# antoyang/TubeDETR

Hardware: AMD Instinct MI355X
Metric: training clips/sec (fwd+bwd) at T=100 k=4 res=352, 1/2/4/8 MI355X (higher is better)
Workload: dtype bf16

## Files before the change

### tubedetr_amd/csrc/gemm_conv.hip

```cpp
#include <stdlib.h>

#include "gemm_dev.h"
#include "gemm_host.h"

#ifndef TD_BIG_XCD_CONTIG
#define TD_BIG_XCD_CONTIG 1
#endif
namespace td {

struct GemmParams {
  const char* src;
  const char* w;
  char* out;
  td_conv_desc d;
  int M, K;
  uint32_t src_bytes, w_bytes;
  unsigned long long* dbg;
  const float* bias;
  const char* residual;
  const char* mask_src;
  int relu, sigmoid;
  float alpha;
  uint32_t drop_thresh;
  float drop_scale;
// ... 933 lines not shown
      const int row = it * RPI + rsub;
      const int sw = row & (CPRW - 1);
      float v[EPL];
#pragma unroll
      for (int q = 0; q < EPL / 4; ++q) {
        const float4 f = *(const float4*)(stg + row * WN + (((cc * (EPL / 4) + q) ^ sw) * 4));
        v[4 * q + 0] = f.x + bias[4 * q + 0]; v[4 * q + 1] = f.y + bias[4 * q + 1];
        v[4 * q + 2] = f.z + bias[4 * q + 2]; v[4 * q + 3] = f.w + bias[4 * q + 3];
      }
      if (p.residual) {
        float r8[EPL];
        unpack16<T>(res[b][it], r8);
#pragma unroll
        for (int r = 0; r < EPL; ++r) v[r] += r8[r];
      }
      if (p.relu) {
#pragma unroll
        for (int r = 0; r < EPL; ++r) v[r] = fmaxf(v[r], 0.f);
      }
      if (p.mask_src) {
        float m8[EPL];
        unpack16<T>(msk[b][it], m8);
#pragma unroll
        for (int r = 0; r < EPL; ++r) v[r] = m8[r] > 0.f ? v[r] : 0.f;
      }
      if (live[b][it]) st16(p.out + offs[b][it] * ES, pack16<T>(v));
    }
    asm volatile("s_waitcnt lgkmcnt(0)" ::: "memory");
  }
  TD_STAMP(5);
#undef TD_STAMP
}

template <int NKT, bool RES, bool MSK>
__global__ __launch_bounds__(256, 2) void pw_resident2_kernel(GemmParams p, int MT, int P) {
  using T = u16;
  constexpr int ES = 2;
  constexpr uint32_t OOB = 0xFFFFFFF0u;
  constexpr int WM = 32, WN = 64, TM = 2, TN = 4;
  constexpr int CPRW = WN / 4, EPL = 8, LPR = WN / EPL, RPI = 64 / LPR, NIT = WM / RPI;
  constexpr int NOPS = NIT * ((RES ? 1 : 0) + (MSK ? 1 : 0));
  constexpr bool AHEAD = NOPS > 0 && !(RES && MSK && NKT == 4);
  constexpr int NA = 2 * NKT;
  constexpr int AUX_NT = (TD_NT & 2) ? 2 : 0;
  __shared__ __attribute__((aligned(16))) char sA0[32768];
  __shared__ __attribute__((aligned(16))) char sA1[32768];
  __shared__ __attribute__((aligned(16))) char sT[4 * 16 * WN * 4];
  const td_conv_desc& d = p.d;
  const int t = threadIdx.x;
  const int wave = __builtin_amdgcn_readfirstlane(t >> 6), lane = t & 63;
  const int NT = d.Nc >> 7;
  const int xcd = blockIdx.x & 7, local = blockIdx.x >> 3;
  const int GPX = P / NT;
  const int nt = local % NT, gl = local / NT;
  if (gl >= GPX) return;
  const int gid = xcd * GPX + gl, G = 8 * GPX;
  const int lrow = lane >> 3, chunk = (lane & 7) ^ lrow;
  const uint32_t out_bytes = (uint32_t)p.M * (uint32_t)d.ldc * ES;
  const __amdgpu_buffer_rsrc_t rs_src = __builtin_amdgcn_make_buffer_rsrc((void*)p.src, 0, p.src_bytes, 0x00020000);
  const __amdgpu_buffer_rsrc_t rs_out = __builtin_amdgcn_make_buffer_rsrc((void*)p.out, 0, out_bytes, 0x00020000);
  const __amdgpu_buffer_rsrc_t rs_res = __builtin_amdgcn_make_buffer_rsrc((void*)(RES ? p.residual : p.out), 0, out_bytes, 0x00020000);
  const __amdgpu_buffer_rsrc_t rs_msk = __builtin_amdgcn_make_buffer_rsrc((void*)(MSK ? p.mask_src : p.out), 0, out_bytes, 0x00020000);
  const int n0 = nt * 128;
  const int HoWo = d.Ho * d.Wo;
  const bool strided = d.stride != 1;
  auto issue_A = [&](char* buf, int mt) {
    const int m0 = mt * 64;
// ... 60 lines not shown
#pragma unroll
      for (int j = 0; j < TM; ++j) acc[i][j] = f32x4{0.f, 0.f, 0.f, 0.f};
#pragma unroll
    for (int kt = 0; kt < NKT; ++kt)
#pragma unroll
      for (int ks = 0; ks < 2; ++ks) {
        const int cidx = ks * 4 + lg;
        uint4 af[TM];
#pragma unroll
        for (int j = 0; j < TM; ++j) {
          const int row = wy * WM + j * 16 + lr;
          af[j] = *(const uint4*)(cur + kt * 8192 + row * 128 + ((cidx ^ (row & 7)) << 4));
        }
#pragma unroll
        for (int i = 0; i < TN; ++i)
#pragma unroll
          for (int j = 0; j < TM; ++j) Mfma<T>::run(wfr[kt][ks][i], af[j], acc[i][j]);
      }
    asm volatile("s_waitcnt lgkmcnt(0)" ::: "memory");
    __builtin_amdgcn_s_barrier();
    issue_A(cur, mt + 2 * G);
    if constexpr (AHEAD) fetch_ops(mt + G, B ^ 1);
    if constexpr (NOPS > 0) {
      wait_vmcnt<NA + (AHEAD ? NOPS : 0)>();
      __builtin_amdgcn_sched_barrier(0);
    }
    constexpr int RB = AHEAD ? B : 0;
#pragma unroll
    for (int j = 0; j < TM; ++j) {
#pragma unroll
      for (int i = 0; i < TN; ++i) {
        const int c = (i * 4 + lg) ^ (lr & (CPRW - 1));
        const f32x4 a = acc[i][j];
        *(float4*)(stg + lr * WN + c * 4) = make_float4(a[0], a[1], a[2], a[3]);
      }
      asm volatile("s_waitcnt lgkmcnt(0)" ::: "memory");
#pragma unroll
      for (int h = 0; h < 16 / RPI; ++h) {
        const int it = j * (16 / RPI) + h;
        const int row = h * RPI + rsub;
        const int sw = row & (CPRW - 1);
        float v[EPL];
#pragma unroll
        for (int q = 0; q < EPL / 4; ++q) {
          const float4 f = *(const float4*)(stg + row * WN + (((cc * (EPL / 4) + q) ^ sw) * 4));
          v[4 * q + 0] = f.x + bias[4 * q + 0]; v[4 * q + 1] = f.y + bias[4 * q + 1];
          v[4 * q + 2] = f.z + bias[4 * q + 2]; v[4 * q + 3] = f.w + bias[4 * q + 3];
        }
        const uint32_t off = seg_off(mt, it);
        if constexpr (RES) {
          float r8[EPL];
          unpack16<T>(make_uint4(res[RB][it].x, res[RB][it].y, res[RB][it].z, res[RB][it].w), r8);
#pragma unroll
          for (int r = 0; r < EPL; ++r) v[r] += r8[r];
        }
        if (p.relu) {
#pragma unroll
          for (int r = 0; r < EPL; ++r) v[r] = fmaxf(v[r], 0.f);
        }
        if constexpr (MSK) {
          float m8[EPL];
          unpack16<T>(make_uint4(msk[RB][it].x, msk[RB][it].y, msk[RB][it].z, msk[RB][it].w), m8);
#pragma unroll
          for (int r = 0; r < EPL; ++r) v[r] = m8[r] > 0.f ? v[r] : 0.f;
        }
        if (p.drop_thresh) {
#pragma unroll
// ... 4 lines not shown
      }
      asm volatile("s_waitcnt lgkmcnt(0)" ::: "memory");
    }
  };

  int mt = gid;
  issue_A(sA0, mt);
  issue_A(sA1, mt + G);
  if constexpr (AHEAD) fetch_ops(mt, 0);
  while (mt < MT) {
    step(sA0, sA1, mt, ic<0>{});
    mt += G;
    if (mt >= MT) break;
    step(sA1, sA0, mt, ic<1>{});
    mt += G;
  }
  asm volatile("s_waitcnt vmcnt(0)" ::: "memory");
}

}

using namespace td;


static thread_local unsigned long long* g_dbg = nullptr;
extern "C" int td_debug_set_stamp_buffer(unsigned long long* buf) { g_dbg = buf; return TD_OK; }
unsigned long long* td::stamp_buffer() { return g_dbg; }

const GemmKnobs& td::gemm_knobs() {
  static const GemmKnobs knobs = [] {
    GemmKnobs k;
    const struct { const char* name; int* value; } vars[] = {
        {"TD_PW_PERSIST", &k.pw_persist}, {"TD_PW_PERSIST_MIN", &k.pw_persist_min}, {"TD_PW_PERSIST_DROPOUT", &k.pw_persist_dropout},
        {"TD_CONV_TAP_UNIFORM", &k.conv_tap_uniform}, {"TD_CONV_BIG", &k.conv_big}, {"TD_CONV_BIG_MIN_WG", &k.conv_big_min_wg},
        {"TD_CONV_TAP_INNER", &k.conv_tap_inner}, {"TD_CONV_BIG_PERSIST", &k.conv_big_persist}, {"TD_CONV_DEEP", &k.conv_deep},
        {"TD_DGRAD_S2_PARITY", &k.dgrad_s2_parity}, {"TD_WGRAD_BLOCKS", &k.wgrad_blocks}, {"TD_WGRAD_WIDE", &k.wgrad_wide},
        {"TD_WGRAD_WIDE_MIN_M", &k.wgrad_wide_min_m}, {"TD_WGRAD_SPLIT_STAGES", &k.wgrad_split_stages}};
    for (const auto& v : vars)
      if (const char* e = getenv(v.name)) *v.value = atoi(e);
    return k;
  }();
  return knobs;
}

static int fill_epilogue(GemmParams& p, const td_epilogue* e, const char* who) {
  p.alpha = 1.f;
  if (!e) return TD_OK;
  p.bias = e->bias;
  p.residual = (const char*)e->residual;
  p.mask_src = (const char*)e->mask_src;
  p.relu = e->relu;
  p.sigmoid = e->sigmoid;
  if (e->alpha != 0.f) p.alpha = e->alpha;
  if (e->dropout_p > 0.f) {
    TD_REQUIRE(e->dropout_p < 1.f, "%s: dropout_p must be < 1", who);
    p.drop_thresh = dropout_threshold(e->dropout_p);
    p.drop_scale = 1.f / (1.f - e->dropout_p);
    p.seed = e->dropout_seed;
    p.seed_dev = e->dropout_counter;
  }
  return TD_OK;
}

typedef void (*GemmKernel)(GemmParams);
typedef void (*PersistentKernel)(GemmParams, int, int);
template <typename T, int BM, int BN, int NST>
static GemmKernel tiled_instance(int walk) {
  switch (walk) {
    case TD_GEMM_WALK_POINTWISE: return conv_gemm_kernel<T, BM, BN, NST, true>;
    case TD_GEMM_WALK_TAP_UNIFORM: return conv_gemm_kernel<T, BM, BN, NST, false, true>;
    case TD_GEMM_WALK_GATHER: return conv_gemm_kernel<T, BM, BN, NST, false>;
    default: return conv_gemm_kernel<T, BM, BN, 2, true, false, true>;
  }
}
template <int NKT>
static PersistentKernel persistent_instance(bool res, bool msk) {
  if (res) return msk ? pw_resident2_kernel<NKT, true, true> : pw_resident2_kernel<NKT, true, false>;
  return msk ? pw_resident2_kernel<NKT, false, true> : pw_resident2_kernel<NKT, false, false>;
}

static int launch_route(const GemmRoute& r, GemmParams& p, hipStream_t st) {
  const bool bf16 = r.dtype == TD_BF16, tu = r.walk == TD_GEMM_WALK_TAP_UNIFORM;
  GemmKernel k = nullptr;
  PersistentKernel kp = nullptr;
  switch (r.kernel) {
    case TD_GEMM_KERNEL_PERSISTENT:
      kp = r.nkt == 1 ? persistent_instance<1>(r.res, r.msk) : r.nkt == 2 ? persistent_instance<2>(r.res, r.msk) :
           r.nkt == 3 ? persistent_instance<3>(r.res, r.msk) : persistent_instance<4>(r.res, r.msk);
      break;
    case TD_GEMM_KERNEL_BIG8:
      if (tu) k = r.res ? conv_gemm_big8_kernel<true, true> : conv_gemm_big8_kernel<true, false>;
      else k = r.res ? conv_gemm_big8_kernel<false, true> : conv_gemm_big8_kernel<false, false>;
      break;
    case TD_GEMM_KERNEL_BIG8N: k = tu ? conv_gemm_big8n_kernel<true> : conv_gemm_big8n_kernel<false>; break;
    default:
      if (r.bn == 64) k = bf16 ? tiled_instance<u16, 128, 64, 2>(r.walk) : tiled_instance<float, 128, 64, 2>(r.walk);
      else if (r.stages == 3) k = tiled_instance<u16, 64, 128, 3>(r.walk);
      else if (r.bm == 64) k = bf16 ? tiled_instance<u16, 64, 128, 2>(r.walk) : tiled_instance<float, 64, 128, 2>(r.walk);
      else k = bf16 ? tiled_instance<u16, 128, 128, 2>(r.walk) : tiled_instance<float, 128, 128, 2>(r.walk);
  }
  const bool prof = prof_on();
  if (prof) {
    prof_begin(r.family, r.dtype, 2.0 * r.M * r.N * r.K, st, r.M, r.N, r.K, r.R, r.stride, r.mode);
    prof_set_bytes(r.bytes);
  }
  if (kp) kp<<<r.grid, r.block, 0, st>>>(p, r.MTp, r.Pp);
  else k<<<r.grid, r.block, 0, st>>>(p);
  if (prof) prof_end(st);
  return check_launch(r.label);
}

static int conv_gemm_launch(const void* src, const void* wmat, void* out, const td_conv_desc* d, const td_epilogue* e, int dtype, int n_cu,
                            const WeightSubset* sub, td_stream_t stream, td_gemm_route* report) {
  GemmRoute r;
  int rc = plan_conv_launch(d, epi_flags(e), dtype, n_cu, gemm_knobs(), sub, r);
  if (rc) return rc;
  GemmParams p;
  memset(&p, 0, sizeof(p));
  rc = fill_epilogue(p, e, "td_conv_gemm");
  if (rc) return rc;
  if (report) {
// ... 21 lines not shown

static int conv_gemm_call(const void* src, const void* wmat, void* out, const td_conv_desc* d, const td_epilogue* e, int dtype, int n_cu,
                          td_stream_t stream, td_gemm_route* report, int* n_report) {
  const bool split = conv_splits_by_parity(d, e, dtype, gemm_knobs());
  if (n_report) *n_report = split ? 4 : 1;
  if (!split) return conv_gemm_launch(src, wmat, out, d, e, dtype, n_cu, nullptr, stream, report);
  int rc = validate(d, dtype, "td_conv_gemm");
  for (int i = 0; i < 4 && !rc; ++i) {
    const ParityClass c = parity_class(d, i >> 1, i & 1);
    td_epilogue ec;
    memset(&ec, 0, sizeof(ec));
    if (e) ec = *e;
    if (ec.residual) ec.residual = (const char*)ec.residual + c.out_off;
    if (ec.mask_src) ec.mask_src = (const char*)ec.mask_src + c.out_off;
    if (report) rc = conv_gemm_launch(nullptr, nullptr, nullptr, &c.d, &ec, dtype, n_cu, &c.sub, stream, report + i);
    else rc = conv_gemm_launch(src, (const char*)wmat + c.w_off, (char*)out + c.out_off, &c.d, &ec, dtype, n_cu, &c.sub, stream, nullptr);
  }
  return rc;
}

extern "C" int td_conv_gemm(const void* src, const void* wmat, void* out, const td_conv_desc* d, const td_epilogue* e,
                            int dtype, td_stream_t stream) {
  TD_REQUIRE(src && wmat && out && d, "td_conv_gemm: null pointer");
  return conv_gemm_call(src, wmat, out, d, e, dtype, cu_count(), stream, nullptr, nullptr);
}

extern "C" int td_conv_gemm_route(const td_conv_desc* d, const td_epilogue* e, int dtype, int n_cu, td_gemm_route* routes, int* n_routes) {
  TD_REQUIRE(d && routes && n_routes, "td_conv_gemm: null pointer");
  TD_REQUIRE(n_cu >= 1, "td_conv_gemm_route: n_cu=%d", n_cu);
  return conv_gemm_call(nullptr, nullptr, nullptr, d, e, dtype, n_cu, nullptr, routes, n_routes);
}

static int linear_ex_call(const void* a1, const void* a2, const void* wmat, void* out, const td_linear_ex_desc* x, bool has_a2, const td_epilogue* e,
                          int dtype, td_stream_t stream, td_gemm_route* report) {
  GemmRoute r;
  int rc = plan_linear_ex(x, has_a2, epi_flags(e), dtype, r);
  if (rc) return rc;
  GemmParams p;
  memset(&p, 0, sizeof(p));
  rc = fill_epilogue(p, e, "td_linear_ex");
  if (rc) return rc;
  if (report) {
    *report = r;
    return TD_OK;
  }
  p.src = (const char*)a1;
  p.src2 = (const char*)a2;
  p.w = (const char*)wmat;
  p.out = (char*)out;
  p.M = r.M;
  p.K = r.K;
  p.K1 = x->K1;
  p.lda1 = x->lda1;
  p.lda2 = a2 ? x->lda2 : 0;
  p.ldr = x->ldr > 0 ? x->ldr : x->ldc;
  p.w_shared = (a2 && x->w_shared) ? 1 : 0;
  p.a1_map = x->a1_map;
  p.a2_map = a2 ? x->a2_map : nullptr;
  p.out_map = x->out_map;
  p.res_map = x->res_map;
  p.d.N = 1; p.d.Hs = x->M; p.d.Ws = 1; p.d.C = p.K; p.d.Ho = x->M; p.d.Wo = 1; p.d.R = p.d.S = 1; p.d.stride = 1; p.d.Nc = x->N; p.d.ldc = x->ldc; p.d.out_sp = 1;
  p.src_bytes = r.src_bytes;
  p.src2_bytes = r.src2_bytes;
  p.w_bytes = r.w_bytes;
  return launch_route(r, p, (hipStream_t)stream);
}

extern "C" int td_linear_ex(const void* a1, const void* a2, const void* wmat, void* out, const td_linear_ex_desc* x, const td_epilogue* e,
                            int dtype, td_stream_t stream) {
  TD_REQUIRE(a1 && wmat && out && x, "td_linear_ex: null pointer");
  return linear_ex_call(a1, a2, wmat, out, x, a2 != nullptr, e, dtype, stream, nullptr);
}

extern "C" int td_linear_ex_route(const td_linear_ex_desc* x, int has_a2, const td_epilogue* e, int dtype, int n_cu, td_gemm_route* routes, int* n_routes) {
  TD_REQUIRE(x && routes && n_routes, "td_linear_ex: null pointer");
  (void)n_cu;
  *n_routes = 1;
  return linear_ex_call(nullptr, nullptr, nullptr, nullptr, x, has_a2 != 0, e, dtype, nullptr, routes);
}
```

### tubedetr_amd/csrc/gemm_route.h

```cpp
#pragma once
#include <stdint.h>
#include <string.h>

#include "../../include/tubedetr_hip.h"

#ifndef TD_REQUIRE
namespace td {
void set_error(const char* fmt, ...);
inline int cdiv(int a, int b) { return (a + b - 1) / b; }
}
#define TD_REQUIRE(cond, ...)           \
  do {                                  \
    if (!(cond)) {                      \
      td::set_error(__VA_ARGS__);       \
      return TD_ERR_INVALID;            \
    }                                   \
  } while (0)
#endif

namespace td {

struct GemmKnobs {
  int pw_persist = 1;
  int pw_persist_min = 4;
  int pw_persist_dropout = 1;
  int conv_tap_uniform = 1;
  int conv_big = 1;
  int conv_big_min_wg = 160;
  int conv_tap_inner = 1;
  int conv_big_persist = 1;
  int conv_deep = 1;
  int dgrad_s2_parity = 1;
  int wgrad_blocks = 256, wgrad_wide = 1, wgrad_wide_min_m = 4096, wgrad_split_stages = 0;
};

struct WeightSubset {
  int w_ld;
  int ntap;
  int wtap[4];
  size_t w_bytes;
};

struct EpiFlags {
  bool res, msk, sigmoid, drop;
  float alpha;
};
inline EpiFlags epi_flags(const td_epilogue* e) {
  EpiFlags f = {false, false, false, false, 1.f};
  if (e) f = {e->residual != nullptr, e->mask_src != nullptr, e->sigmoid != 0, e->dropout_p > 0.f, e->alpha != 0.f ? e->alpha : 1.f};
  return f;
}

struct GemmRoute : td_gemm_route {
  bool res, msk;
  int nkt, MTp, Pp;
  int tap_inner;
  uint32_t src_bytes, src2_bytes, w_bytes;
  double bytes;
  const char* label;
};

inline int validate(const td_conv_desc* d, int dtype, const char* who) {
  const int vec = dtype == TD_BF16 ? 8 : 4;
  TD_REQUIRE(dtype == TD_F32 || dtype == TD_BF16, "%s: bad dtype %d", who, dtype);
  TD_REQUIRE(d->C % vec == 0, "%s: source channels C=%d must be a multiple of %d (pad them)", who, d->C, vec);
  TD_REQUIRE(d->N > 0 && d->Hs > 0 && d->Ws > 0 && d->Ho > 0 && d->Wo > 0 && d->R > 0 && d->S > 0 && d->stride > 0,
             "%s: bad geometry", who);
  TD_REQUIRE((double)d->N * d->Hs * d->Ws * d->C < 2147483647.0, "%s: source tensor exceeds 2^31 elements", who);
  TD_REQUIRE(!d->aniso || (d->mode == 0 && d->stride_w >= 1 && d->pad_w >= 0 && d->out_sp <= 1), "%s: anisotropic stride / padding is a forward-only geometry", who);
  return TD_OK;
}

inline void tiled_shape(GemmRoute& r) {
  const bool narrow = r.N <= 64;
  const int tiles128 = cdiv(r.M, 128) * cdiv(r.N, 128);
  const bool small_m = !narrow && (tiles128 < 512 || r.K <= 512);
  r.kernel = TD_GEMM_KERNEL_TILED;
  r.family = narrow ? TD_PROF_GEMM_128x64 : (small_m ? TD_PROF_GEMM_64x128 : TD_PROF_GEMM_128x128);
  r.bm = small_m ? 64 : 128;
  r.bn = narrow ? 64 : 128;
  r.stages = 2;
  r.grid = 8 * cdiv(cdiv(r.M, r.bm), 8) * cdiv(r.N, r.bn);
  r.block = 256;
}

inline int plan_conv_launch(const td_conv_desc* d, const EpiFlags& f, int dtype, int n_cu, const GemmKnobs& kn, const WeightSubset* sub, GemmRoute& r) {
  int rc = validate(d, dtype, "td_conv_gemm");
// ... 66 lines not shown
  return TD_OK;
}

inline bool conv_splits_by_parity(const td_conv_desc* d, const td_epilogue* e, int dtype, const GemmKnobs& kn) {
  return kn.dgrad_s2_parity && dtype == TD_BF16 && d->mode == 1 && d->stride == 2 && d->R == 3 && d->S == 3 && d->pad == 1 && !d->aniso && d->out_sp <= 1 &&
         d->Ho == 2 * d->Hs && d->Wo == 2 * d->Ws && d->C % 64 == 0 && d->ldc >= d->Nc && !(e && (e->dropout_p > 0.f || e->sigmoid));
}
struct ParityClass {
  td_conv_desc d;
  WeightSubset sub;
  size_t w_off, out_off;
};
inline ParityClass parity_class(const td_conv_desc* d, int ph, int pw) {
  const int Hg = d->Hs, Wg = d->Ws, Co = d->C, H = d->Ho, W = d->Wo;
  const size_t es = 2, wbytes = (size_t)d->Nc * 9 * Co * es;
  const int nr = ph ? 2 : 1, ns = pw ? 2 : 1;
  const int rmap[2] = {ph ? 2 : 1, 0}, smap[2] = {pw ? 2 : 1, 0};
  ParityClass c;
  memset(&c, 0, sizeof(c));
  c.d = {d->N, Hg, Wg, Co, Hg, Wg, nr, ns, 1, 0, 0, d->Nc, d->ldc, 2, H, W};
  c.sub.w_ld = 9 * Co;
  c.sub.ntap = nr * ns;
  for (int r = 0; r < nr; ++r)
    for (int s_ = 0; s_ < ns; ++s_) c.sub.wtap[r * ns + s_] = rmap[r] * 3 + smap[s_];
  c.out_off = ((size_t)ph * W + pw) * d->ldc * es;
  if (c.sub.ntap == 1) {
    c.w_off = (size_t)c.sub.wtap[0] * Co * es;
    c.sub.wtap[0] = 0;
  }
  c.sub.w_bytes = wbytes - c.w_off;
  return c;
}

inline int plan_linear_ex(const td_linear_ex_desc* x, bool has_a2, const EpiFlags& f, int dtype, GemmRoute& r) {
  TD_REQUIRE(dtype == TD_F32 || dtype == TD_BF16, "td_linear_ex: bad dtype %d", dtype);
  const int vec = dtype == TD_BF16 ? 8 : 4, bk = dtype == TD_BF16 ? 64 : 32;
  const int es = dtype == TD_BF16 ? 2 : 4;
  const int K2 = has_a2 ? x->K2 : 0;
  TD_REQUIRE(x->M >= 1 && x->N >= 1 && x->K1 >= vec && K2 >= 0, "td_linear_ex: bad sizes");
  TD_REQUIRE(x->K1 % vec == 0 && K2 % vec == 0 && x->lda1 % vec == 0 && (!has_a2 || x->lda2 % vec == 0), "td_linear_ex: K1 / K2 / lda must be multiples of %d", vec);
  TD_REQUIRE(!has_a2 || x->K1 % bk == 0, "td_linear_ex: with a second source K1=%d must be a multiple of the K tile (%d)", x->K1, bk);
  TD_REQUIRE(x->lda1 >= x->K1 && (!has_a2 || x->lda2 >= K2) && x->ldc >= x->N, "td_linear_ex: row stride smaller than the row");
  TD_REQUIRE(x->rows1 >= 1 && (!has_a2 || x->rows2 >= 1) && (x->a1_map || x->rows1 >= x->M) && (!has_a2 || x->a2_map || x->rows2 >= x->M),
             "td_linear_ex: source has fewer rows than M and no row map");
  const bool w_shared = has_a2 && x->w_shared;
  TD_REQUIRE(!w_shared || K2 == x->K1, "td_linear_ex: a shared weight needs K2 == K1");
  memset(&r, 0, sizeof(r));
  r.dtype = dtype; r.M = x->M; r.N = x->N; r.K = x->K1 + K2; r.R = 1; r.stride = 1; r.mode = 2;
  const double b1 = (double)x->rows1 * x->lda1 * es, b2 = has_a2 ? (double)x->rows2 * x->lda2 * es : 16.0, wb = (double)x->N * (w_shared ? x->K1 : r.K) * es;
  TD_REQUIRE(b1 < 4294967000.0 && b2 < 4294967000.0 && wb < 4294967000.0, "td_linear_ex: operand exceeds the 4 GiB buffer-descriptor range");
  r.src_bytes = (uint32_t)b1;
  r.src2_bytes = (uint32_t)b2;
  r.w_bytes = (uint32_t)wb;
  r.res = f.res;
  r.msk = f.msk;
  tiled_shape(r);
  r.walk = TD_GEMM_WALK_GX;
  r.bytes = ((double)r.M * r.K + (double)r.N * r.K + (double)r.M * r.N * (1 + f.res + f.msk)) * es;
  r.label = "td_linear_ex";
  return TD_OK;
}

}
```

### tubedetr_amd/csrc/resnet_exec.hip

```cpp
#include <stdlib.h>

#include <algorithm>
#include <vector>

#include "td_common.h"

namespace td {

struct ConvSpec {
  int cin, cout, k, stride, pad;
};
struct Tens {
  size_t off;
  int H, W, C;
};
struct BlockPlan {
  int conv[4];
  int stride, stage;
  Tens in, h1, h2, idt, out;
};
struct Plan {
  std::vector<ConvSpec> convs;
  std::vector<BlockPlan> blocks;
  Tens x, stem, pool;
// ... 64 lines not shown
      t->off = off;
      off += bytes(*t);
    } else {
      t->off = (size_t)(ring % 6) * maxb;
      ++ring;
    }
  }
  P.total = save ? off : 6 * maxb;
  Tens prev = P.pool;
  for (auto& b : P.blocks) {
    b.in = prev;
    prev = b.out;
  }
  return P;
}

struct FrameGroups {
  double lim_elems;
  int N;
  FrameGroups(int N_, int H, int W, int es) : N(N_) {
    lim_elems = std::min(2147483647.0, 4294963200.0 / es);
    if (const char* e = getenv("TD_TRUNK_MAX_FRAMES")) lim_elems = std::min(lim_elems, atof(e) * 16.0 * H * W);
  }
  int step(size_t per_frame) const {
    const long long nmax = std::max(1LL, (long long)(lim_elems / (double)per_frame));
    if (N <= nmax) return N;
    const long long groups = (N + nmax - 1) / nmax;
    return (int)((N + groups - 1) / groups);
  }
};
static inline size_t frame_elems(const Tens& t) { return (size_t)t.H * t.W * t.C; }

static int run_conv(const char* ws, const Tens& in, const Tens& out, int N, const ConvSpec& c, const void* w, const float* bias,
                    const char* residual, int relu, int dtype, td_stream_t st, const FrameGroups* fg = nullptr) {
  const int es = dtype == TD_BF16 ? 2 : 4;
  const int step = fg ? fg->step(std::max(frame_elems(in), frame_elems(out))) : N;
  for (int f0 = 0; f0 < N; f0 += step) {
    const int n = std::min(step, N - f0);
    td_conv_desc d = {n, in.H, in.W, in.C, out.H, out.W, c.k, c.k, c.stride, c.pad, 0, c.cout, c.cout, 1, 0, 0};
    td_epilogue e;
    memset(&e, 0, sizeof(e));
    e.bias = bias;
    e.residual = residual ? residual + (size_t)f0 * frame_elems(out) * es : nullptr;
    e.relu = relu;
    int rc = td_conv_gemm(ws + in.off + (size_t)f0 * frame_elems(in) * es, w, (void*)(ws + out.off + (size_t)f0 * frame_elems(out) * es), &d, &e, dtype, st);
    if (rc) return rc;
  }
  return TD_OK;
}

}
using namespace td;

extern "C" size_t td_resnet_fwd_ws_bytes(int N, int H, int W, const int* nblocks, int dtype, int save) {
  return make_plan(N, H, W, nblocks, dtype, save).total;
}

extern "C" int td_resnet_num_convs(const int* nblocks) {
  int n = 1;
  for (int s = 0; s < 4; ++s) n += 3 * nblocks[s] + (nblocks[s] > 0 ? 1 : 0);
  return n;
}

extern "C" int td_resnet_fwd(const td_frame_source* srcs, int n_srcs, const float* mean, const float* inv_std, int N, int H, int W,
                             const int* nblocks, const void* const* w_fwd, const float* const* bias, int save, void* ws,
                             size_t ws_bytes, void** feat, int* feat_hw, int stem_pairs, int first_train_stage, int dtype, td_stream_t stream) {
  TD_REQUIRE(srcs && n_srcs >= 1 && nblocks && w_fwd && bias && ws && feat, "td_resnet_fwd: null pointer");
  TD_REQUIRE(dtype == TD_F32 || dtype == TD_BF16, "td_resnet_fwd: bad dtype");
  {
    long long tot = 0;
    for (int i = 0; i < n_srcs; ++i) tot += srcs[i].n;
    TD_REQUIRE(tot == N, "td_resnet_fwd: the sources contribute %lld frames, N = %d", tot, N);
  }
  Plan P = make_plan(N, H, W, nblocks, dtype, save);
  TD_REQUIRE(ws_bytes >= P.total, "td_resnet_fwd: workspace too small (%zu < %zu)", ws_bytes, P.total);
  char* base = (char*)ws;
  int rc;
  const FrameGroups groups(N, H, W, P.es);
  const FrameGroups* fg = save ? nullptr : &groups;
  bool stem_done = false;
  if (stem_pairs) {
    TD_REQUIRE(dtype == TD_BF16 && (W & 1) == 0, "td_resnet_fwd: the pixel-pair stem needs bf16 and an even frame width");
    rc = td_frames_to_nhwc(srcs, n_srcs, 3, H, W, 4, mean, inv_std, base + P.x.off, dtype, stream);
    if (rc) return rc;
    static const int fused = [] { const char* e_ = getenv("TD_STEM_FUSED"); return e_ ? atoi(e_) : 1; }();
    if (fused) {
      rc = td_stem_pool(base + P.x.off, w_fwd[0], bias[0], base + P.pool.off, N, H, W, dtype, stream);
      stem_done = true;
    } else {
      const int step = fg ? fg->step(frame_elems(P.stem)) : N;
      for (int f0 = 0; f0 < N && !rc; f0 += step) {
        td_conv_desc d = {std::min(step, N - f0), H, W / 2, 8, P.stem.H, P.stem.W, 7, 4, 2, 3, 0, 64, 64, 1, 0, 0, 1, 1, 2};
        td_epilogue e;
        memset(&e, 0, sizeof(e));
        e.bias = bias[0];
        e.relu = 1;
        rc = td_conv_gemm(base + P.x.off + (size_t)f0 * H * W * 4 * P.es, w_fwd[0], base + P.stem.off + (size_t)f0 * frame_elems(P.stem) * P.es, &d, &e, dtype, stream);
      }
    }
  } else {
    rc = td_frames_to_nhwc(srcs, n_srcs, 3, H, W, P.x.C, mean, inv_std, base + P.x.off, dtype, stream);
    if (rc) return rc;
    rc = run_conv(base, P.x, P.stem, N, P.convs[0], w_fwd[0], bias[0], nullptr, 1, dtype, stream, fg);
  }
  if (rc) return rc;
  if (!stem_done) {
    const int step = fg ? fg->step(frame_elems(P.stem)) : N;
    for (int f0 = 0; f0 < N; f0 += step)
      if ((rc = td_maxpool3x3s2(base + P.stem.off + (size_t)f0 * frame_elems(P.stem) * P.es, base + P.pool.off + (size_t)f0 * frame_elems(P.pool) * P.es,
                                std::min(step, N - f0), P.stem.H, P.stem.W, 64, dtype, stream)))
        return rc;
  }
  static const int l1_fused = [] { const char* e = getenv("TD_L1_FUSED"); return e ? atoi(e) : 2; }();
  static const int chain_on = [] { const char* e = getenv("TD_CHAIN"); return e ? atoi(e) : 1; }();
  bool h1_done = false;
  for (size_t bi = 0; bi < P.blocks.size(); ++bi) {
    auto& b = P.blocks[bi];
    const int c1 = b.conv[0], c2 = b.conv[1], c3 = b.conv[2], cd = b.conv[3];
    if (l1_fused && (l1_fused >= 2 || cd >= 0) && dtype == TD_BF16 && (!save || b.stage < first_train_stage) && b.stride == 1 && P.convs[c1].cout == 64 &&
        P.convs[c3].cout == 256 && ((P.convs[c1].cin == 64 && cd >= 0) || (P.convs[c1].cin == 256 && cd < 0)) &&
        (fg || (double)N * b.out.H * b.out.W * 256 < 2147483647.0)) {
      const int step = fg ? fg->step(frame_elems(b.out)) : N;
      for (int f0 = 0; f0 < N; f0 += step)
        if ((rc = td_bottleneck_fused(base + b.in.off + (size_t)f0 * frame_elems(b.in) * P.es, base + b.out.off + (size_t)f0 * frame_elems(b.out) * P.es, w_fwd[c1],
                                      bias[c1], w_fwd[c2], bias[c2], w_fwd[c3], bias[c3], cd >= 0 ? w_fwd[cd] : nullptr, cd >= 0 ? bias[cd] : nullptr,
                                      std::min(step, N - f0), b.in.H, b.in.W, P.convs[c1].cin, dtype, stream)))
          return rc;
      continue;
    }
    if (!h1_done && (rc = run_conv(base, b.in, b.h1, N, P.convs[c1], w_fwd[c1], bias[c1], nullptr, 1, dtype, stream, fg))) return rc;
    h1_done = false;
    if ((rc = run_conv(base, b.h1, b.h2, N, P.convs[c2], w_fwd[c2], bias[c2], nullptr, 1, dtype, stream, fg))) return rc;
    const char* idt = base + b.in.off;
    if (cd >= 0) {
      if ((rc = run_conv(base, b.in, b.idt, N, P.convs[cd], w_fwd[cd], bias[cd], nullptr, 0, dtype, stream, fg))) return rc;
      idt = base + b.idt.off;
    }
    if (chain_on && dtype == TD_BF16 && bi + 1 < P.blocks.size() && P.blocks[bi + 1].stage == b.stage && P.convs[c3].cin == 256 && P.convs[c3].cout == 1024 &&
        P.blocks[bi + 1].stride == 1 && (double)N * b.out.H * b.out.W * 1024.0 * 2.0 < 4294967000.0) {
      const BlockPlan& nb_ = P.blocks[bi + 1];
      const int n1 = nb_.conv[0];
      if ((rc = td_pw_chain2(base + b.h2.off, w_fwd[c3], bias[c3], idt, base + b.out.off, w_fwd[n1], bias[n1], base + nb_.h1.off, N * b.out.H * b.out.W, 256, dtype, stream)))
        return rc;
      h1_done = true;
      continue;
    }
    if ((rc = run_conv(base, b.h2, b.out, N, P.convs[c3], w_fwd[c3], bias[c3], idt, 1, dtype, stream, fg))) return rc;
  }
  const Tens& last = P.blocks.empty() ? P.pool : P.blocks.back().out;
  *feat = base + last.off;
  if (feat_hw) {
    feat_hw[0] = last.H;
    feat_hw[1] = last.W;
    feat_hw[2] = last.C;
  }
  return TD_OK;
}

static size_t dwk_bytes(const Plan& P, int first_stage, std::vector<size_t>* offs) {
  size_t off = 0;
  if (offs) offs->assign(P.convs.size(), (size_t)-1);
  for (auto& b : P.blocks) {
    if (b.stage < first_stage) continue;
    for (int q = 0; q < 4; ++q) {
      int ci = b.conv[q];
      if (ci < 0) continue;
      const ConvSpec& c = P.convs[ci];
      if (offs) (*offs)[ci] = off;
      off += align256((size_t)c.cout * c.k * c.k * c.cin * sizeof(float));
    }
  }
  return off;
}
static size_t grad_slot_bytes(const Plan& P, int N, int first_stage) {
  size_t m = 0;
  for (auto& b : P.blocks) {
    if (b.stage < first_stage) continue;
    for (const Tens* t : {&b.in, &b.h1, &b.h2, &b.out}) m = std::max(m, align256((size_t)N * t->H * t->W * t->C * P.es));
  }
  return m;
}

static bool wgrad_batched() {
// ... 157 lines not shown
```

### tubedetr_amd/models/backbone.py

```python
from __future__ import annotations

import os

from collections import OrderedDict
from typing import List

import torch
from torch import nn
from torch.autograd import Function

from .. import ops
from ..functional import prepared
from ..util.misc import NestedTensor
from .position_encoding import build_position_encoding

RESNET_LAYERS = {"resnet50": (3, 4, 6, 3), "resnet101": (3, 4, 23, 3)}


class FrozenBatchNorm2d(nn.Module):

    def __init__(self, n: int):
        super().__init__()
        self.register_buffer("weight", torch.ones(n))
        self.register_buffer("bias", torch.zeros(n))
# ... 102 lines not shown
        self._split = None
        if leaf.grad is None:
            return
        ctx = feat.grad_fn
        assert ctx is not None and hasattr(ctx, "dims"), "backward_trunk_iter: the trunk pass kept nothing for backward"
        first = None
        for name, blk in self.blocks():
            if blk.conv1.weight.requires_grad:
                first = int(name[5]) - 1
                break
        by_w = {id(p): p for p in self.trainable_weights()}
        for stage in range(3, (4 if first is None else first) - 1, -1):
            with torch.no_grad():
                got = ResNetTrunkFn._enqueue(ctx, leaf.grad, stage)
                ws_ = []
                for wid, g in got.items():
                    p = by_w[wid]
                    p.grad = g if p.grad is None else p.grad.add_(g)
                    ws_.append(p)
            yield stage, ws_


def _prep(conv: ConvWeight, bn: FrozenBatchNorm2d, dt, need_dgrad, cpad=None):
    return prepared(conv.weight, dt, bn=bn.fold(), need_dgrad=need_dgrad, cpad=cpad)


def _conv_list(body: "ResNetBody"):
    out = [(body.conv1, body.bn1)]
    for _, blk in body.blocks():
        out += [(blk.conv1, blk.bn1), (blk.conv2, blk.bn2), (blk.conv3, blk.bn3)]
        if blk.downsample is not None:
            out.append((blk.downsample[0], blk.downsample[1]))
    return out


def _ptr_array(tensors):
    import ctypes as C

    return (C.c_void_p * len(tensors))(*[t.data_ptr() if t is not None else None for t in tensors])


class ResNetTrunkFn(Function):

    @staticmethod
    def forward(ctx, body: "ResNetBody", x: torch.Tensor, dt: torch.dtype, n_grad: int, *trainable):
        import ctypes as C

        from .. import _hip

        from ..util.misc import FrameSources

        L = _hip.lib()
        code = _hip.dtype_code(dt)
        vec = ops.vec_of(dt)
        save = 1 if len(trainable) > 0 else 0
        if not isinstance(x, FrameSources):
            x = x.detach()
            x = FrameSources([((x if x.dtype == torch.uint8 else x.float()).contiguous(), None)])
        assert len(x.shape) == 4 and x.shape[1] == 3, "frames must be (N,3,H,W)"
        N, _, H, W = x.shape
        mean = inv_std = None
        if x.dtype == torch.uint8:
            mean = (C.c_float * 3)(*body.pixel_mean)
            inv_std = (C.c_float * 3)(*[1.0 / v for v in body.pixel_std])
        convs = _conv_list(body)
        preps = [prepared(c.weight, dt, bn=bn.fold(), need_dgrad=c.weight.requires_grad, cpad=vec if i == 0 else None)
# ... 27 lines not shown
                    fs.valid_hw = vhw.data_ptr() if vhw is not None else None
                else:
                    fs.data, fs.index = t.data_ptr() + lo * t.stride(0) * t.element_size(), None
                    fs.valid_hw = vhw.data_ptr() + 8 * lo if vhw is not None else None
                out.append(fs)
            arr = (_hip.FrameSource * len(out))(*out)
            return arr, len(out)

        n_max = 4 * ResNetBody.max_frames(H, W, dt)
        n_chunks = 1 if save else -(-N // n_max)
        if n_chunks > 1:
            step_n = -(-N // n_chunks)
            full, hw = None, (C.c_int * 3)()
            assert n_grad == N or not save
            for a in range(0, N, step_n):
                b = min(N, a + step_n)
                srcs, n_srcs = sources(a, b)
                nbytes = L.td_resnet_fwd_ws_bytes(b - a, H, W, nb, code, 0)
                ws = torch.empty(nbytes, dtype=torch.uint8, device=x.device)
                feat_p = C.c_void_p()
                _hip.check(L.td_resnet_fwd(srcs, n_srcs, mean, inv_std, b - a, H, W, nb, _ptr_array(w_ptrs), _ptr_array([p[2] for p in preps]),
                                           0, ws.data_ptr(), nbytes, C.byref(feat_p), hw, int(pairs), first_stage, code, _hip.stream_ptr()), "td_resnet_fwd")
                off = feat_p.value - ws.data_ptr()
                n_el = (b - a) * hw[0] * hw[1] * hw[2]
                if full is None:
                    full = torch.empty((N, hw[0], hw[1], hw[2]), dtype=dt, device=x.device)
                full[a:b].copy_(ws[off : off + n_el * dt.itemsize].view(dt).view(b - a, hw[0], hw[1], hw[2]))
            return full[:n_grad], full[n_grad:]
        srcs, n_srcs = sources(0, N)
        nbytes = L.td_resnet_fwd_ws_bytes(N, H, W, nb, code, save)
        ws = torch.empty(nbytes, dtype=torch.uint8, device=x.device)
        feat_p = C.c_void_p()
        hw = (C.c_int * 3)()
        _hip.check(L.td_resnet_fwd(srcs, n_srcs, mean, inv_std, N, H, W, nb, _ptr_array(w_ptrs), _ptr_array([p[2] for p in preps]),
                                   save, ws.data_ptr(), nbytes, C.byref(feat_p), hw, int(pairs), first_stage, code, _hip.stream_ptr()), "td_resnet_fwd")
        off = feat_p.value - ws.data_ptr()
        n_el = N * hw[0] * hw[1] * hw[2]
        feat = ws[off : off + n_el * dt.itemsize].view(dt).view(N, hw[0], hw[1], hw[2])
        if not save:
            feat = feat.clone()
            return feat[:n_grad], feat[n_grad:]
        ctx.body, ctx.dt, ctx.ws, ctx.preps, ctx.dims = body, dt, ws, preps, (n_grad, N, H, W)
        a, b = feat[:n_grad], feat[n_grad:]
        ctx.mark_non_differentiable(b)
        return a, b

    @staticmethod
    def _enqueue(ctx, dfeat, only_stage=-1):
        import ctypes as C

        from .. import _hip, ops

        body, dt, ws, preps = ctx.body, ctx.dt, ctx.ws, ctx.preps
        N, N_fwd, H, W = ctx.dims
        L = _hip.lib()
        code = _hip.dtype_code(dt)
        convs = _conv_list(body)
        first_stage = 4
        for name, blk in body.blocks():
            if blk.conv1.weight.requires_grad:
                first_stage = int(name[5]) - 1
                break
        nb = (C.c_int * 4)(*body.layers)
        st = getattr(ctx, "bwd_state", None)
        if st is None:
            sizes = [c.weight.numel() if c.weight.requires_grad else 0 for c, _ in convs]
            offs_ = [0]
            for n_ in sizes:
# ... 119 lines not shown
```

### tubedetr_amd/ops.py

```python
from __future__ import annotations

import os

import ctypes as C
from typing import Optional, Tuple

import torch

from . import _hip
from ._hip import ConvDesc, Epilogue, check, dtype_code, ptr, stream_ptr

Tensor = torch.Tensor


class _ZeroArena:

    def __init__(self, chunk: int):
        self.chunk = chunk
        self.buf = None
        self.off = 0

    def take(self, shape, device) -> torch.Tensor:
        n = 1
        for d_ in shape:
# ... 206 lines not shown
        return
    key0 = (jobs[0][0].dtype, jobs[0][0].device)
    if any((j[0].dtype, j[0].device) != key0 for j in jobs):
        groups: dict = {}
        for j in jobs:
            groups.setdefault((j[0].dtype, j[0].device), []).append(j)
        for sub in groups.values():
            linear_wgrad_batch(sub)
        return
    arr = (_hip.WgradJob * len(jobs))()
    for a, job in zip(arr, jobs):
        g, x, dw_ptr, db_ptr = job[:4]
        M, K = x.shape
        Nn = g.shape[1]
        assert g.shape[0] == M and g.stride(1) == 1 and x.is_contiguous() and g.dtype == x.dtype
        a.g, a.src, a.dW, a.scale, a.dbias = g.data_ptr(), x.data_ptr(), dw_ptr, None, db_ptr
        a.d = _desc(1, M, 1, K, M, 1, 1, 1, 1, 0, 0, Nn, Nn)
        a.ldg, a.ci_real = g.stride(0), K
        a.accumulate = int(len(job) > 4 and bool(job[4]))
    nbytes = _hip.lib().td_conv_wgrad_batch_table_bytes(len(jobs))
    dev = jobs[0][0].device
    th, td_, done = job_tables.take(nbytes, dev)
    check(_hip.lib().td_conv_wgrad_batch(arr, len(jobs), dtype_code(jobs[0][0].dtype), th.data_ptr(), td_.data_ptr(), nbytes, stream_ptr()),
          "td_conv_wgrad_batch(linears)")
    done()


def linear_fwd(x: Tensor, w: Tensor, bias: Optional[Tensor] = None, *, residual=None, relu=False, sigmoid=False,
               mask_src=None, dropout_p=0.0, seed=0, alpha=1.0, out: Optional[Tensor] = None) -> Tensor:
    M, K = x.shape
    Nn = w.shape[0]
    assert w.shape[1] == K and w.dtype == x.dtype and x.is_contiguous() and w.is_contiguous()
    y = out if out is not None else torch.empty((M, Nn), dtype=x.dtype, device=x.device)
    conv_gemm_raw(x, w, y, _desc(1, M, 1, K, M, 1, 1, 1, 1, 0, 0, Nn, Nn), _epi(bias, residual, mask_src, relu, sigmoid, dropout_p, seed, alpha))
    return y


def pw_chain2(y2: Tensor, w3: Tensor, b3: Tensor, residual: Tensor, w1: Tensor, b1: Tensor, *, out: Optional[Tensor] = None,
              h1: Optional[Tensor] = None) -> Tuple[Tensor, Tensor]:
    M, P = y2.shape
    assert y2.dtype == torch.bfloat16 and w3.shape == (4 * P, P) and w1.shape == (P, 4 * P) and residual.shape == (M, 4 * P)
    assert y2.is_contiguous() and w3.is_contiguous() and w1.is_contiguous() and residual.is_contiguous()
    assert b3.dtype == torch.float32 and b1.dtype == torch.float32 and b3.numel() == 4 * P and b1.numel() == P
    out = out if out is not None else torch.empty((M, 4 * P), dtype=y2.dtype, device=y2.device)
    h1 = h1 if h1 is not None else torch.empty((M, P), dtype=y2.dtype, device=y2.device)
    check(_hip.lib().td_pw_chain2(ptr(y2), ptr(w3), ptr(b3), ptr(residual), ptr(out), ptr(w1), ptr(b1), ptr(h1), M, P, dtype_code(y2.dtype),
                                  stream_ptr()), "td_pw_chain2")
    return out, h1


def _rows2d(t: Tensor):
    assert t.dim() == 2 and t.stride(1) == 1, "row-major 2-D operand expected (unit column stride)"
    return t


def linear_ex(a1: Tensor, w: Tensor, bias: Optional[Tensor] = None, *, a2: Optional[Tensor] = None, a1_map: Optional[Tensor] = None,
              a2_map: Optional[Tensor] = None, w_shared: bool = False, out: Optional[Tensor] = None, out_map: Optional[Tensor] = None,
              out_rows: Optional[int] = None, residual: Optional[Tensor] = None, res_map: Optional[Tensor] = None, relu=False, mask_src=None,
              dropout_p=0.0, seed=0, alpha=1.0) -> Tensor:
    _rows2d(a1)
    K1 = a1.shape[1]
    K2 = _rows2d(a2).shape[1] if a2 is not None else 0
    M = int(a1_map.numel()) if a1_map is not None else a1.shape[0]
    Nn = w.shape[0]
    assert w.is_contiguous() and w.dtype == a1.dtype and w.shape[1] == (K1 if (w_shared or a2 is None) else K1 + K2)
    for m_ in (a1_map, a2_map, out_map, res_map):
        assert m_ is None or (m_.dtype == torch.int32 and m_.is_contiguous() and m_.numel() == M)
    if out is None:
# ... 328 lines not shown
```

Before: 106.3.

## Route small-K dense linears to persistent weight-resident kernel; write trunk features in place

Adds a route in plan_linear_ex that sends dense bf16 linears with K<=256 and N a multiple of 128 to the persistent weight-resident pointwise kernel, with a new ALPHA template variant that applies the scaling factor. The Python linear_fwd caches a per-shape routing decision and calls td_linear_ex when the conv path would not already pick the persistent kernel. Separately, the non-saving ResNet forward now writes its last block directly into a caller-allocated feature tensor, which removes the workspace-to-output clone. Risks are the extra template instantiations and cached routing keyed on alpha and epilogue flags.

Result: no change. 106.8 (median of 6 runs) (+0.5%).

```diff
diff --git a/tubedetr_amd/csrc/gemm_conv.hip b/tubedetr_amd/csrc/gemm_conv.hip
--- a/tubedetr_amd/csrc/gemm_conv.hip
+++ b/tubedetr_amd/csrc/gemm_conv.hip
@@ -989,7 +989,7 @@
 #undef TD_STAMP
 }
 
-template <int NKT, bool RES, bool MSK>
+template <int NKT, bool RES, bool MSK, bool ALPHA = false>
 __global__ __launch_bounds__(256, 2) void pw_resident2_kernel(GemmParams p, int MT, int P) {
   using T = u16;
   constexpr int ES = 2;
@@ -1116,7 +1116,8 @@
       for (int i = 0; i < TN; ++i) {
         const int c = (i * 4 + lg) ^ (lr & (CPRW - 1));
         const f32x4 a = acc[i][j];
-        *(float4*)(stg + lr * WN + c * 4) = make_float4(a[0], a[1], a[2], a[3]);
+        if constexpr (ALPHA) *(float4*)(stg + lr * WN + c * 4) = make_float4(a[0] * p.alpha, a[1] * p.alpha, a[2] * p.alpha, a[3] * p.alpha);
+        else *(float4*)(stg + lr * WN + c * 4) = make_float4(a[0], a[1], a[2], a[3]);
       }
       asm volatile("s_waitcnt lgkmcnt(0)" ::: "memory");
 #pragma unroll
@@ -1187,7 +1188,7 @@
     GemmKnobs k;
     const struct { const char* name; int* value; } vars[] = {
         {"TD_PW_PERSIST", &k.pw_persist}, {"TD_PW_PERSIST_MIN", &k.pw_persist_min}, {"TD_PW_PERSIST_DROPOUT", &k.pw_persist_dropout},
-        {"TD_CONV_TAP_UNIFORM", &k.conv_tap_uniform}, {"TD_CONV_BIG", &k.conv_big}, {"TD_CONV_BIG_MIN_WG", &k.conv_big_min_wg},
+        {"TD_LINEAR_WS", &k.linear_ws}, {"TD_LINEAR_WS_MIN", &k.linear_ws_min}, {"TD_CONV_TAP_UNIFORM", &k.conv_tap_uniform}, {"TD_CONV_BIG", &k.conv_big}, {"TD_CONV_BIG_MIN_WG", &k.conv_big_min_wg},
         {"TD_CONV_TAP_INNER", &k.conv_tap_inner}, {"TD_CONV_BIG_PERSIST", &k.conv_big_persist}, {"TD_CONV_DEEP", &k.conv_deep},
         {"TD_DGRAD_S2_PARITY", &k.dgrad_s2_parity}, {"TD_WGRAD_BLOCKS", &k.wgrad_blocks}, {"TD_WGRAD_WIDE", &k.wgrad_wide},
         {"TD_WGRAD_WIDE_MIN_M", &k.wgrad_wide_min_m}, {"TD_WGRAD_SPLIT_STAGES", &k.wgrad_split_stages}};
@@ -1233,6 +1234,11 @@
   if (res) return msk ? pw_resident2_kernel<NKT, true, true> : pw_resident2_kernel<NKT, true, false>;
   return msk ? pw_resident2_kernel<NKT, false, true> : pw_resident2_kernel<NKT, false, false>;
 }
+template <int NKT>
+static PersistentKernel persistent_alpha_instance(bool res, bool msk) {
+  if (res) return msk ? pw_resident2_kernel<NKT, true, true, true> : pw_resident2_kernel<NKT, true, false, true>;
+  return msk ? pw_resident2_kernel<NKT, false, true, true> : pw_resident2_kernel<NKT, false, false, true>;
+}
 
 static int launch_route(const GemmRoute& r, GemmParams& p, hipStream_t st) {
   const bool bf16 = r.dtype == TD_BF16, tu = r.walk == TD_GEMM_WALK_TAP_UNIFORM;
@@ -1240,8 +1246,10 @@
   PersistentKernel kp = nullptr;
   switch (r.kernel) {
     case TD_GEMM_KERNEL_PERSISTENT:
-      kp = r.nkt == 1 ? persistent_instance<1>(r.res, r.msk) : r.nkt == 2 ? persistent_instance<2>(r.res, r.msk) :
-           r.nkt == 3 ? persistent_instance<3>(r.res, r.msk) : persistent_instance<4>(r.res, r.msk);
+      if (r.scaled) kp = r.nkt == 1 ? persistent_alpha_instance<1>(r.res, r.msk) : r.nkt == 2 ? persistent_alpha_instance<2>(r.res, r.msk) :
+                         r.nkt == 3 ? persistent_alpha_instance<3>(r.res, r.msk) : persistent_alpha_instance<4>(r.res, r.msk);
+      else kp = r.nkt == 1 ? persistent_instance<1>(r.res, r.msk) : r.nkt == 2 ? persistent_instance<2>(r.res, r.msk) :
+                r.nkt == 3 ? persistent_instance<3>(r.res, r.msk) : persistent_instance<4>(r.res, r.msk);
       break;
     case TD_GEMM_KERNEL_BIG8:
       if (tu) k = r.res ? conv_gemm_big8_kernel<true, true> : conv_gemm_big8_kernel<true, false>;
@@ -1329,9 +1337,9 @@
 }
 
 static int linear_ex_call(const void* a1, const void* a2, const void* wmat, void* out, const td_linear_ex_desc* x, bool has_a2, const td_epilogue* e,
-                          int dtype, td_stream_t stream, td_gemm_route* report) {
+                          int dtype, int n_cu, td_stream_t stream, td_gemm_route* report) {
   GemmRoute r;
-  int rc = plan_linear_ex(x, has_a2, epi_flags(e), dtype, r);
+  int rc = plan_linear_ex(x, has_a2, epi_flags(e), dtype, n_cu, gemm_knobs(), r);
   if (rc) return rc;
   GemmParams p;
   memset(&p, 0, sizeof(p));
@@ -1366,12 +1374,11 @@
 extern "C" int td_linear_ex(const void* a1, const void* a2, const void* wmat, void* out, const td_linear_ex_desc* x, const td_epilogue* e,
                             int dtype, td_stream_t stream) {
   TD_REQUIRE(a1 && wmat && out && x, "td_linear_ex: null pointer");
-  return linear_ex_call(a1, a2, wmat, out, x, a2 != nullptr, e, dtype, stream, nullptr);
+  return linear_ex_call(a1, a2, wmat, out, x, a2 != nullptr, e, dtype, cu_count(), stream, nullptr);
 }
 
 extern "C" int td_linear_ex_route(const td_linear_ex_desc* x, int has_a2, const td_epilogue* e, int dtype, int n_cu, td_gemm_route* routes, int* n_routes) {
   TD_REQUIRE(x && routes && n_routes, "td_linear_ex: null pointer");
-  (void)n_cu;
   *n_routes = 1;
-  return linear_ex_call(nullptr, nullptr, nullptr, nullptr, x, has_a2 != 0, e, dtype, nullptr, routes);
-}
+  return linear_ex_call(nullptr, nullptr, nullptr, nullptr, x, has_a2 != 0, e, dtype, n_cu, nullptr, routes);
+}
diff --git a/tubedetr_amd/csrc/gemm_route.h b/tubedetr_amd/csrc/gemm_route.h
--- a/tubedetr_amd/csrc/gemm_route.h
+++ b/tubedetr_amd/csrc/gemm_route.h
@@ -24,6 +24,8 @@
   int pw_persist = 1;
   int pw_persist_min = 4;
   int pw_persist_dropout = 1;
+  int linear_ws = 1;
+  int linear_ws_min = 4;
   int conv_tap_uniform = 1;
   int conv_big = 1;
   int conv_big_min_wg = 160;
@@ -53,6 +55,7 @@
 
 struct GemmRoute : td_gemm_route {
   bool res, msk;
+  bool scaled;
   int nkt, MTp, Pp;
   int tap_inner;
   uint32_t src_bytes, src2_bytes, w_bytes;
@@ -185,7 +188,7 @@
   return c;
 }
 
-inline int plan_linear_ex(const td_linear_ex_desc* x, bool has_a2, const EpiFlags& f, int dtype, GemmRoute& r) {
+inline int plan_linear_ex(const td_linear_ex_desc* x, bool has_a2, const EpiFlags& f, int dtype, int n_cu, const GemmKnobs& kn, GemmRoute& r) {
   TD_REQUIRE(dtype == TD_F32 || dtype == TD_BF16, "td_linear_ex: bad dtype %d", dtype);
   const int vec = dtype == TD_BF16 ? 8 : 4, bk = dtype == TD_BF16 ? 64 : 32;
   const int es = dtype == TD_BF16 ? 2 : 4;
@@ -207,6 +210,28 @@
   r.w_bytes = (uint32_t)wb;
   r.res = f.res;
   r.msk = f.msk;
+  {
+    const bool dense = !has_a2 && !x->a1_map && !x->a2_map && !x->out_map && !x->res_map && x->lda1 == x->K1 && (!f.res || x->ldr <= 0 || x->ldr == x->ldc);
+    const int NTp = x->N / 128, Pp = 2 * n_cu / 8;
+    const bool shape_ok = dense && dtype == TD_BF16 && x->K1 % 64 == 0 && x->K1 <= 256 && x->N % 128 == 0 &&
+                          (NTp == 1 || NTp == 2 || NTp == 4 || NTp == 8 || NTp == 16) && Pp >= NTp && x->ldc % 8 == 0 && !f.sigmoid && n_cu % 8 == 0 &&
+                          (double)x->M * x->ldc < 2147483000.0;
+    const int MTp = cdiv(x->M, 64);
+    const int groups = shape_ok ? 8 * (Pp / NTp) : 1;
+    if (kn.linear_ws && shape_ok && MTp >= kn.linear_ws_min * groups) {
+      r.kernel = TD_GEMM_KERNEL_PERSISTENT;
+      r.family = TD_PROF_PW_RESIDENT;
+      r.bm = 64; r.bn = 128;
+      r.walk = TD_GEMM_WALK_POINTWISE;
+      r.scaled = f.alpha != 1.f;
+      r.nkt = x->K1 / 64; r.MTp = MTp; r.Pp = Pp;
+      r.grid = 2 * n_cu;
+      r.block = 256;
+      r.bytes = ((double)r.M * r.K + (double)r.N * r.K + (double)r.M * r.N * (1 + f.res + f.msk)) * es;
+      r.label = "td_linear_ex(pw_resident)";
+      return TD_OK;
+    }
+  }
   tiled_shape(r);
   r.walk = TD_GEMM_WALK_GX;
   r.bytes = ((double)r.M * r.K + (double)r.N * r.K + (double)r.M * r.N * (1 + f.res + f.msk)) * es;
diff --git a/tubedetr_amd/csrc/resnet_exec.hip b/tubedetr_amd/csrc/resnet_exec.hip
--- a/tubedetr_amd/csrc/resnet_exec.hip
+++ b/tubedetr_amd/csrc/resnet_exec.hip
@@ -120,9 +120,10 @@
 static inline size_t frame_elems(const Tens& t) { return (size_t)t.H * t.W * t.C; }
 
 static int run_conv(const char* ws, const Tens& in, const Tens& out, int N, const ConvSpec& c, const void* w, const float* bias,
-                    const char* residual, int relu, int dtype, td_stream_t st, const FrameGroups* fg = nullptr) {
+                    const char* residual, int relu, int dtype, td_stream_t st, const FrameGroups* fg = nullptr, char* out_at = nullptr) {
   const int es = dtype == TD_BF16 ? 2 : 4;
   const int step = fg ? fg->step(std::max(frame_elems(in), frame_elems(out))) : N;
+  char* const dst = out_at ? out_at : (char*)ws + out.off;
   for (int f0 = 0; f0 < N; f0 += step) {
     const int n = std::min(step, N - f0);
     td_conv_desc d = {n, in.H, in.W, in.C, out.H, out.W, c.k, c.k, c.stride, c.pad, 0, c.cout, c.cout, 1, 0, 0};
@@ -131,7 +132,7 @@
     e.bias = bias;
     e.residual = residual ? residual + (size_t)f0 * frame_elems(out) * es : nullptr;
     e.relu = relu;
-    int rc = td_conv_gemm(ws + in.off + (size_t)f0 * frame_elems(in) * es, w, (void*)(ws + out.off + (size_t)f0 * frame_elems(out) * es), &d, &e, dtype, st);
+    int rc = td_conv_gemm(ws + in.off + (size_t)f0 * frame_elems(in) * es, w, dst + (size_t)f0 * frame_elems(out) * es, &d, &e, dtype, st);
     if (rc) return rc;
   }
   return TD_OK;
@@ -163,6 +164,7 @@
   Plan P = make_plan(N, H, W, nblocks, dtype, save);
   TD_REQUIRE(ws_bytes >= P.total, "td_resnet_fwd: workspace too small (%zu < %zu)", ws_bytes, P.total);
   char* base = (char*)ws;
+  char* const feat_at = (!save && !P.blocks.empty()) ? (char*)*feat : nullptr;
   int rc;
   const FrameGroups groups(N, H, W, P.es);
   const FrameGroups* fg = save ? nullptr : &groups;
@@ -205,12 +207,13 @@
   for (size_t bi = 0; bi < P.blocks.size(); ++bi) {
     auto& b = P.blocks[bi];
     const int c1 = b.conv[0], c2 = b.conv[1], c3 = b.conv[2], cd = b.conv[3];
+    char* const out_at = (feat_at && bi + 1 == P.blocks.size()) ? feat_at : nullptr;
     if (l1_fused && (l1_fused >= 2 || cd >= 0) && dtype == TD_BF16 && (!save || b.stage < first_train_stage) && b.stride == 1 && P.convs[c1].cout == 64 &&
         P.convs[c3].cout == 256 && ((P.convs[c1].cin == 64 && cd >= 0) || (P.convs[c1].cin == 256 && cd < 0)) &&
         (fg || (double)N * b.out.H * b.out.W * 256 < 2147483647.0)) {
       const int step = fg ? fg->step(frame_elems(b.out)) : N;
       for (int f0 = 0; f0 < N; f0 += step)
-        if ((rc = td_bottleneck_fused(base + b.in.off + (size_t)f0 * frame_elems(b.in) * P.es, base + b.out.off + (size_t)f0 * frame_elems(b.out) * P.es, w_fwd[c1],
+        if ((rc = td_bottleneck_fused(base + b.in.off + (size_t)f0 * frame_elems(b.in) * P.es, (out_at ? out_at : base + b.out.off) + (size_t)f0 * frame_elems(b.out) * P.es, w_fwd[c1],
                                       bias[c1], w_fwd[c2], bias[c2], w_fwd[c3], bias[c3], cd >= 0 ? w_fwd[cd] : nullptr, cd >= 0 ? bias[cd] : nullptr,
                                       std::min(step, N - f0), b.in.H, b.in.W, P.convs[c1].cin, dtype, stream)))
           return rc;
@@ -233,10 +236,10 @@
       h1_done = true;
       continue;
     }
-    if ((rc = run_conv(base, b.h2, b.out, N, P.convs[c3], w_fwd[c3], bias[c3], idt, 1, dtype, stream, fg))) return rc;
+    if ((rc = run_conv(base, b.h2, b.out, N, P.convs[c3], w_fwd[c3], bias[c3], idt, 1, dtype, stream, fg, out_at))) return rc;
   }
   const Tens& last = P.blocks.empty() ? P.pool : P.blocks.back().out;
-  *feat = base + last.off;
+  *feat = feat_at ? feat_at : base + last.off;
   if (feat_hw) {
     feat_hw[0] = last.H;
     feat_hw[1] = last.W;
diff --git a/tubedetr_amd/models/backbone.py b/tubedetr_amd/models/backbone.py
--- a/tubedetr_amd/models/backbone.py
+++ b/tubedetr_amd/models/backbone.py
@@ -158,6 +158,19 @@
         if blk.downsample is not None:
             out.append((blk.downsample[0], blk.downsample[1]))
     return out
+
+
+def _feat_dims(H: int, W: int, layers):
+    def co(v, k, s, p):
+        return (v + 2 * p - k) // s + 1
+
+    h, w, c = co(co(H, 7, 2, 3), 3, 2, 1), co(co(W, 7, 2, 3), 3, 2, 1), 64
+    for s, n in enumerate(layers):
+        if n:
+            if s > 0:
+                h, w = co(h, 3, 2, 1), co(w, 3, 2, 1)
+            c = 256 << s
+    return h, w, c
 
 
 def _ptr_array(tensors):
@@ -251,8 +264,15 @@
         ws = torch.empty(nbytes, dtype=torch.uint8, device=x.device)
         feat_p = C.c_void_p()
         hw = (C.c_int * 3)()
+        result = None
+        if not save and any(body.layers) and os.environ.get("TD_TRUNK_FEAT_INPLACE", "1") != "0":
+            result = torch.empty((N,) + _feat_dims(H, W, body.layers), dtype=dt, device=x.device)
+            feat_p = C.c_void_p(result.data_ptr())
         _hip.check(L.td_resnet_fwd(srcs, n_srcs, mean, inv_std, N, H, W, nb, _ptr_array(w_ptrs), _ptr_array([p[2] for p in preps]),
                                    save, ws.data_ptr(), nbytes, C.byref(feat_p), hw, int(pairs), first_stage, code, _hip.stream_ptr()), "td_resnet_fwd")
+        if result is not None:
+            assert feat_p.value == result.data_ptr() and tuple(hw) == tuple(result.shape[1:]), "td_resnet_fwd: features not where they were asked for"
+            return result[:n_grad], result[n_grad:]
         off = feat_p.value - ws.data_ptr()
         n_el = N * hw[0] * hw[1] * hw[2]
         feat = ws[off : off + n_el * dt.itemsize].view(dt).view(N, hw[0], hw[1], hw[2])
diff --git a/tubedetr_amd/ops.py b/tubedetr_amd/ops.py
--- a/tubedetr_amd/ops.py
+++ b/tubedetr_amd/ops.py
@@ -262,8 +262,40 @@
     Nn = w.shape[0]
     assert w.shape[1] == K and w.dtype == x.dtype and x.is_contiguous() and w.is_contiguous()
     y = out if out is not None else torch.empty((M, Nn), dtype=x.dtype, device=x.device)
-    conv_gemm_raw(x, w, y, _desc(1, M, 1, K, M, 1, 1, 1, 1, 0, 0, Nn, Nn), _epi(bias, residual, mask_src, relu, sigmoid, dropout_p, seed, alpha))
-    return y
+    desc, epi = _desc(1, M, 1, K, M, 1, 1, 1, 1, 0, 0, Nn, Nn), _epi(bias, residual, mask_src, relu, sigmoid, dropout_p, seed, alpha)
+    if _linear_on_ws_route(x, M, Nn, K, desc, epi):
+        xd = _dense_linear_desc(M, Nn, K)
+        check(_hip.lib().td_linear_ex(ptr(x), None, ptr(w), ptr(y), C.byref(xd), C.byref(epi), dtype_code(x.dtype), stream_ptr()), "td_linear_ex")
+        return y
+    conv_gemm_raw(x, w, y, desc, epi)
+    return y
+
+
+def _dense_linear_desc(M: int, Nn: int, K: int) -> "_hip.LinearExDesc":
+    xd = _hip.LinearExDesc()
+    xd.M, xd.N, xd.K1, xd.lda1, xd.ldc, xd.ldr, xd.rows1 = M, Nn, K, K, Nn, Nn, M
+    return xd
+
+
+_WS_ROUTE: dict = {}
+_CU_COUNT: dict = {}
+
+
+def _linear_on_ws_route(x: Tensor, M: int, Nn: int, K: int, desc: ConvDesc, epi: Epilogue) -> bool:
+    if x.dtype != torch.bfloat16 or K > 256 or K % 64 or Nn % 128 or not x.is_cuda:
+        return False
+    dev = x.device.index if x.device.index is not None else torch.cuda.current_device()
+    key = (dev, M, Nn, K, bool(epi.bias), bool(epi.residual), bool(epi.mask_src), epi.relu, epi.sigmoid, epi.dropout_p > 0, epi.alpha)
+    hit = _WS_ROUTE.get(key)
+    if hit is None:
+        n_cu = _CU_COUNT.get(dev)
+        if n_cu is None:
+            n_cu = _CU_COUNT[dev] = torch.cuda.get_device_properties(dev).multi_processor_count
+        hit = False
+        if conv_gemm_route(desc, epi, x.dtype, n_cu)[0].kernel != _hip.TD_GEMM_KERNEL_PERSISTENT:
+            hit = linear_ex_route(_dense_linear_desc(M, Nn, K), False, epi, x.dtype, n_cu)[0].kernel == _hip.TD_GEMM_KERNEL_PERSISTENT
+        _WS_ROUTE[key] = hit
+    return hit
 
 
 def pw_chain2(y2: Tensor, w3: Tensor, b3: Tensor, residual: Tensor, w1: Tensor, b1: Tensor, *, out: Optional[Tensor] = None,
```
